# timmywanttolearn/distributed_model_parallel

Measured on AMD Instinct MI355X. Metric: images/sec (whole node) ResNet-50 DDP bf16, higher is better.
Workload: dtype bf16; 1 GPU; model=resnet50, device=cuda, global_batch=2048, per_gpu_batch=2048, image_size=224, parallelism=ddp1, single_rank_comm=False, ranks=1, rccl_ranks=1, launcher=single, optimizer=FlatSGD(fp32 master), sync_bn=False, channels_last=True, grad_comm=none(world_size=1), hip_graph=False, checkpoint_segments=0

## Files before the change

csrc/api.h:

```cpp
#pragma once

#include <ATen/ATen.h>
#include <c10/util/Optional.h>

#include <cstdint>
#include <string>
#include <vector>

namespace dmp {

bool attention_supported(int64_t S, int64_t head_dim);
void set_attention_variant(int fwd, int bwd);
std::vector<int64_t> get_attention_variant();
void set_attention_long_from(int64_t n);
int64_t get_attention_long_from();
std::vector<at::Tensor> attention_forward(const at::Tensor& qkv, int64_t B, int64_t S, int64_t H, double scale);
at::Tensor attention_backward(const at::Tensor& dout, const at::Tensor& qkv, const at::Tensor& o,
                              const at::Tensor& lse, int64_t B, int64_t S, int64_t H, double scale);

at::Tensor bn_local_moments(const at::Tensor& x, int64_t C);
std::vector<at::Tensor> bn_forward_apply(const at::Tensor& x, const at::Tensor& sums,
                                         const c10::optional<at::Tensor>& weight,
                                         const c10::optional<at::Tensor>& bias,
                                         const c10::optional<at::Tensor>& running_mean,
// ... 92 lines not shown
                                      const c10::optional<at::Tensor>& invstd,
                                      const c10::optional<at::Tensor>& weight,
                                      const c10::optional<at::Tensor>& bias,
                                      const std::vector<int64_t>& res_map,
                                      const c10::optional<at::Tensor>& a2,
                                      const c10::optional<at::Tensor>& ebias,
                                      const std::vector<int64_t>& a2_map);
at::Tensor gemm_tn(const at::Tensor& A, const at::Tensor& B, at::ScalarType out_dtype,
                   const std::vector<int64_t>& b_map, const c10::optional<at::Tensor>& pro_scale,
                   const c10::optional<at::Tensor>& pro_shift, bool a_mapped,
                   const c10::optional<at::Tensor>& out);
std::vector<at::Tensor> conv_nt(const at::Tensor& x, const at::Tensor& wmat, int64_t kh,
                                int64_t kw, int64_t stride, int64_t pad, int64_t ho, int64_t wo,
                                bool transposed, const c10::optional<at::Tensor>& pro_scale,
                                const c10::optional<at::Tensor>& pro_shift,
                                const std::string& mode,
                                const c10::optional<at::Tensor>& epi_scale,
                                const c10::optional<at::Tensor>& epi_shift,
                                const c10::optional<at::Tensor>& residual, bool relu,
                                int64_t kc);
at::Tensor conv_wgrad(const at::Tensor& dy, const at::Tensor& x, int64_t kh, int64_t kw,
                      int64_t stride, int64_t pad, int64_t ho, int64_t wo,
                      at::ScalarType out_dtype, int64_t kc, const c10::optional<at::Tensor>& out);
void set_gemm_tile(int64_t t);
void set_phase_dgrad(bool on);
void set_tn_wide(bool on);

at::Tensor space_to_depth2(const at::Tensor& x, int64_t pad, int64_t out_channels);
at::Tensor pad_channels16(const at::Tensor& x, int64_t pad, int64_t extra_w);

bool stem_halo_supported(int64_t hs, int64_t ws, int64_t ho, int64_t wo);
std::vector<at::Tensor> stem_halo_fwd(const at::Tensor& s, const at::Tensor& wm, int64_t ho, bool moments);
at::Tensor stem_halo_wgrad(const at::Tensor& dy, const at::Tensor& s, int64_t ho, at::ScalarType out_dtype);
at::Tensor stem_fold_finish(const at::Tensor& img, int64_t ho, int64_t wo, const at::Tensor& t_dz,
                            const at::Tensor& t_y, const at::Tensor& sums, const at::Tensor& cnt,
                            const at::Tensor& invstd, const c10::optional<at::Tensor>& weight, const at::Tensor& mean,
                            at::ScalarType out_dtype);

at::Tensor wgrad3x3(const at::Tensor& dy, const at::Tensor& x, int64_t stride);
bool wgrad3x3_supported(int64_t C, int64_t H, int64_t W, int64_t stride);
void set_wgrad3x3_waves(int64_t nw);

at::Tensor batch_mix(const at::Tensor& x, const at::Tensor& perm, double lam, const std::vector<int64_t>& box);

at::Tensor gemm_xl(const at::Tensor& A, const at::Tensor& B, const std::string& mode,
                   const c10::optional<at::Tensor>& bias, const c10::optional<at::Tensor>& aux,
                   const c10::optional<at::Tensor>& residual, const c10::optional<at::Tensor>& out);
std::vector<at::Tensor> gemm_xl_dgelu_bgrad(const at::Tensor& A, const at::Tensor& B, const at::Tensor& aux);
std::vector<at::Tensor> gemm_xl_conv(const at::Tensor& A, const at::Tensor& B, const std::string& mode,
                                     const c10::optional<at::Tensor>& residual,
                                     const c10::optional<at::Tensor>& bn_x,
                                     const c10::optional<at::Tensor>& bn_y,
                                     const c10::optional<at::Tensor>& mean,
                                     const c10::optional<at::Tensor>& invstd,
                                     const c10::optional<at::Tensor>& weight,
                                     const c10::optional<at::Tensor>& bias,
                                     const std::vector<int64_t>& res_map,
                                     const c10::optional<at::Tensor>& a2,
                                     const c10::optional<at::Tensor>& ebias,
                                     const c10::optional<at::Tensor>& scale,
                                     const c10::optional<at::Tensor>& shift, bool relu,
                                     const std::vector<int64_t>& a2_map);
std::vector<at::Tensor> conv_xl(const at::Tensor& x, const at::Tensor& wmat, int64_t kh, int64_t kw,
                                int64_t stride, int64_t pad, int64_t ho, int64_t wo, const std::string& mode,
                                const c10::optional<at::Tensor>& residual, const c10::optional<at::Tensor>& bn_x,
                                const c10::optional<at::Tensor>& bn_y, const c10::optional<at::Tensor>& mean,
// ... 80 lines not shown
```

csrc/bindings.cpp:

```cpp
#include <cmath>
#include <torch/extension.h>
#include <torch/csrc/autograd/variable.h>

#include "api.h"
#include "comm/rccl_comm.h"
#include "ddp/reducer.h"
#include "dp/parallel_apply.h"

namespace py = pybind11;

PYBIND11_MODULE(TORCH_EXTENSION_NAME, m) {
  m.doc() = "MI355X-native runtime: RCCL communicator, DDP reducer, HIP kernels (gfx950)";

  m.def("bn_local_moments", &dmp::bn_local_moments,
        py::call_guard<py::gil_scoped_release>());
  m.def("bn_forward_apply", &dmp::bn_forward_apply, py::arg("x"), py::arg("sums"), py::arg("weight"),
        py::arg("bias"), py::arg("running_mean"), py::arg("running_var"), py::arg("momentum"),
        py::arg("eps"), py::arg("residual"), py::arg("relu"), py::arg("C"),
        py::arg("num_batches_tracked") = py::none(), py::arg("out_moments") = false,
        py::arg("clip") = INFINITY,
        py::call_guard<py::gil_scoped_release>());
  m.def("bn_eval_apply", &dmp::bn_eval_apply, py::arg("x"), py::arg("running_mean"),
        py::arg("running_var"), py::arg("weight"), py::arg("bias"), py::arg("eps"), py::arg("residual"),
        py::arg("relu"), py::arg("C"), py::arg("clip") = INFINITY,
// ... 71 lines not shown
        py::arg("shift"), py::arg("k"), py::arg("s"), py::arg("p"),
        py::call_guard<py::gil_scoped_release>());
  m.def("maxpool2d_bn_backward", &dmp::maxpool2d_bn_backward, py::arg("dy"), py::arg("idx"), py::arg("x"),
        py::arg("scale"), py::arg("shift"), py::arg("mean"), py::arg("k"), py::arg("s"), py::arg("p"),
        py::call_guard<py::gil_scoped_release>());
  m.def("pad_channels16", &dmp::pad_channels16, py::arg("x"), py::arg("pad"), py::arg("extra_w") = 0,
        py::call_guard<py::gil_scoped_release>());
  m.def("space_to_depth2", &dmp::space_to_depth2, py::arg("x"), py::arg("pad"), py::arg("out_channels") = 16,
        py::call_guard<py::gil_scoped_release>());

  m.def("gemm_xl", &dmp::gemm_xl, py::arg("A"), py::arg("B"), py::arg("mode") = "store",
        py::arg("bias") = py::none(), py::arg("aux") = py::none(),
        py::arg("residual") = py::none(), py::arg("out") = py::none(),
        py::call_guard<py::gil_scoped_release>());
  m.def("conv_xl", &dmp::conv_xl, py::arg("x"), py::arg("wmat"), py::arg("kh"), py::arg("kw"),
        py::arg("stride"), py::arg("pad"), py::arg("ho"), py::arg("wo"), py::arg("mode") = "moments",
        py::arg("residual") = py::none(), py::arg("bn_x") = py::none(), py::arg("bn_y") = py::none(),
        py::arg("mean") = py::none(), py::arg("invstd") = py::none(), py::arg("weight") = py::none(),
        py::arg("bias") = py::none(),
        "Implicit-GEMM conv (NHWC gather) on the 256x256 ping-pong MFMA kernel with conv epilogues",
        py::call_guard<py::gil_scoped_release>());
  m.def("stem_halo_supported", &dmp::stem_halo_supported);
  m.def("stem_halo_fwd", &dmp::stem_halo_fwd, py::arg("s"), py::arg("wm"), py::arg("ho"), py::arg("moments") = false,
        "ResNet stem (s2d 4x4 conv, 16 -> 64 ch, Wo = 112) forward: halo-tiled, weights in VGPRs",
        py::call_guard<py::gil_scoped_release>());
  m.def("stem_fold_finish", &dmp::stem_fold_finish, py::arg("img"), py::arg("ho"), py::arg("wo"), py::arg("t_dz"),
        py::arg("t_y"), py::arg("sums"), py::arg("cnt"), py::arg("invstd"), py::arg("weight"), py::arg("mean"),
        py::arg("out_dtype"),
        "folded stem weight gradient: BN-backward coefficients, the 16 window sums of the batch-summed "
        "space-to-depth image, and al t_dz + be t_y + cc cols in one launch",
        py::call_guard<py::gil_scoped_release>());
  m.def("stem_halo_wgrad", &dmp::stem_halo_wgrad, py::arg("dy"), py::arg("s"), py::arg("ho"), py::arg("out_dtype"),
        "ResNet stem weight gradient [64, 256]: halo-tiled, dW in VGPRs",
        py::call_guard<py::gil_scoped_release>());
  m.def("wgrad3x3", &dmp::wgrad3x3, py::arg("dy"), py::arg("x"), py::arg("stride") = 1,
        "dW [C, C, 3, 3] (channels_last) of a 3x3/s1/p1 conv: persistent halo-tiled MFMA kernel",
        py::call_guard<py::gil_scoped_release>());
  m.def("wgrad3x3_supported", &dmp::wgrad3x3_supported, py::arg("C"), py::arg("Ho"), py::arg("Wo"),
        py::arg("stride") = 1);
  m.def("set_wgrad3x3_waves", &dmp::set_wgrad3x3_waves);
  m.def("conv3x3_c64", &dmp::conv3x3_c64, py::arg("x"), py::arg("wmat"), py::arg("moments") = false,
        "3x3/s1/p1 64->64-channel conv (W = 56) on the persistent halo-tiled MFMA kernel; "
        "returns (y [N*H*W, 64], fp64 moments [129] or empty)",
        py::call_guard<py::gil_scoped_release>());
  m.def("conv3x3_c128", &dmp::conv3x3_c128, py::arg("x"), py::arg("wmat"), py::arg("moments") = false,
        "3x3/s1/p1 128->128-channel conv (W = 28, H % 4 == 0) on the persistent halo-tiled MFMA kernel "
        "(Cout split over grid halves, K split over wave pairs); returns (y [N*H*W, 128], fp64 moments [257] or empty)",
        py::call_guard<py::gil_scoped_release>());
  m.def("conv3x3_c128_dgrad_s2", &dmp::conv3x3_c128_dgrad_s2, py::arg("dy"), py::arg("wt"),
        "data gradient of a 3x3/s2/p1 128->128 conv (dy 28 wide) as its four stride phases on the halo kernel; "
        "wt = W.permute(1, 2, 3, 0) as [128, 1152]; returns dx [N*2H*56, 128]",
        py::call_guard<py::gil_scoped_release>());
  m.def("conv3x3_c128_supported", &dmp::conv3x3_c128_supported, py::arg("C"), py::arg("H"), py::arg("W"));
  m.def("conv_xl_dgrad_s2", &dmp::conv_xl_dgrad_s2, py::arg("dy"), py::arg("wph"), py::arg("hi"), py::arg("wi"),
        "data gradient of a 3x3/s2/p1 conv as four stride-phase implicit GEMMs on the ping-pong kernel; "
        "returns dx [N*hi*wi, Cin]",
        py::call_guard<py::gil_scoped_release>());
  m.def("set_bn_streaming", &dmp::set_bn_streaming, py::arg("on"),
        "A/B: non-temporal streaming in the BN apply passes over > 256 MB tensors (default on)");
  m.def("set_pool_generic", &dmp::set_pool_generic, py::arg("on"),
        "A/B: route every max-pool geometry through the runtime-k kernels (default off)");
  m.def("set_tn_xl_rounds", &dmp::set_tn_xl_rounds, py::arg("rounds"));
  m.def("set_gemm_xl_trim_heavy", &dmp::set_gemm_xl_trim_heavy, py::arg("on"),
        "A/B: trimmed (192..240-row) tiles for the PIPE-10 heavy-epilogue GEMMs at any K (default on)");
  m.def("set_tn_narrow", &dmp::set_tn_narrow, py::arg("on"),
        "A/B: 4-wave weight-gradient tiles of 64 / 128 on an output side that narrow (default on)");
// ... 237 lines not shown
```

csrc/conv/stem_halo.hip:

```cpp
#include <torch/extension.h>
#include <ATen/hip/HIPContext.h>
#include "../api.h"
#include "../common.h"
#include "../launch.h"

namespace dmp {
namespace {

using bf16 = __bf16;
using lptr_t = __attribute__((address_space(3))) void*;
using v4i16 = short __attribute__((ext_vector_type(4)));
using lds_v4 = __attribute__((address_space(3))) v4i16;
using i16x8 = short __attribute__((ext_vector_type(8)));

constexpr int kWo = 112, kWs = 115, kC = 16, kCo = 64, kK = 256;
constexpr int kPixB = kC * 2;

__device__ __attribute__((aligned(16))) uint32_t g_stem_zero[4];

__device__ __forceinline__ void glds16(const void* g, const char* lds) {
  const uint32_t l = (uint32_t)(uintptr_t)(lptr_t)lds;
  asm volatile("s_mov_b32 m0, %0\n\ts_nop 0\n\tglobal_load_lds_dwordx4 %1, off"
               :: "s"(__builtin_amdgcn_readfirstlane(l)), "v"(g) : "memory", "m0");
}
// ... 291 lines not shown
#pragma unroll
          for (int u = 0; u < 16; ++u) {
            __builtin_amdgcn_sched_group_barrier(0x100, 1, 0);
            __builtin_amdgcn_sched_group_barrier(0x008, 1, 0);
          }
        }
        __builtin_amdgcn_sched_barrier(0);
      };
      step(std::integral_constant<int, 0>{});
      step(std::integral_constant<int, 1>{});
      step(std::integral_constant<int, 2>{});
      step(std::integral_constant<int, 3>{});
      step(std::integral_constant<int, 4>{});
      step(std::integral_constant<int, 5>{});
      step(std::integral_constant<int, 6>{});
      static_assert(W_KS == 7, "unrolled k-steps");
      cur ^= 1;
    }
  };
  switch (wave) {
    case 0: run(std::integral_constant<int, 0>{}); break;
    case 1: run(std::integral_constant<int, 1>{}); break;
    case 2: run(std::integral_constant<int, 2>{}); break;
    default: run(std::integral_constant<int, 3>{}); break;
  }
  float* pb = part + (int64_t)blockIdx.x * (kCo * kK);
#pragma unroll
  for (int i = 0; i < 4; ++i)
#pragma unroll
    for (int j = 0; j < 4; ++j)
#pragma unroll
      for (int e = 0; e < 4; ++e)
        pb[(16 * i + 4 * g + e) * kK + 64 * wave + 16 * j + (lane & 15)] = acc[i][j][e];
}

template <typename OT>
__global__ __launch_bounds__(256) void partial_sum_kernel(const float* __restrict__ part, int nb, int n,
                                                          OT* __restrict__ out) {
  const int grp = threadIdx.x >> 6, tl = threadIdx.x & 63;
  const int e0 = (blockIdx.x * 64 + tl) * 4;
  f32x4 acc[4] = {};
  if (e0 < n) {
    int b = grp;
    for (; b + 12 < nb; b += 16) {
#pragma unroll
      for (int u = 0; u < 4; ++u) acc[u] += *reinterpret_cast<const f32x4*>(part + (int64_t)(b + 4 * u) * n + e0);
    }
    for (; b < nb; b += 4) acc[0] += *reinterpret_cast<const f32x4*>(part + (int64_t)b * n + e0);
  }
  __shared__ f32x4 red[256];
  red[threadIdx.x] = (acc[0] + acc[1]) + (acc[2] + acc[3]);
  __syncthreads();
  if (grp == 0 && e0 < n) {
    const f32x4 v = ((red[tl] + red[64 + tl]) + red[128 + tl]) + red[192 + tl];
#pragma unroll
    for (int u = 0; u < 4; ++u) out[e0 + u] = (OT)v[u];
  }
}

int num_cus() {
  int dev = 0, cus = 256;
  DMP_HIP_CHECK(hipGetDevice(&dev));
  DMP_HIP_CHECK(hipDeviceGetAttribute(&cus, hipDeviceAttributeMultiprocessorCount, dev));
  return cus;
}

// ... 44 lines not shown
  return {y, mom};
}

at::Tensor stem_halo_wgrad(const at::Tensor& dy, const at::Tensor& s, int64_t ho, at::ScalarType out_dtype) {
  check_s(s, ho);
  const int64_t n = s.size(0), hs = s.size(2);
  TORCH_CHECK(dy.is_cuda() && dy.scalar_type() == at::kBFloat16 && dy.is_contiguous() && dy.dim() == 2 &&
                  dy.size(0) == n * ho * kWo && dy.size(1) == kCo,
              "stem halo wgrad: dy must be contiguous [N*Ho*112, 64] bf16");
  const int tpi = (int)((ho + WR - 1) / WR);
  const int tiles = (int)(n * tpi);
  auto out = at::empty({kCo, kK}, s.options().dtype(out_dtype));
  auto stream = at::hip::getCurrentHIPStream();
  if (tiles == 0) return out.zero_();
  const int grid = std::min(tiles, num_cus());
  auto part = at::empty({(int64_t)grid * kCo * kK}, s.options().dtype(at::kFloat));
  hipLaunchKernelGGL(stem_wgrad_kernel, dim3(grid), dim3(256), 0, stream,
                     reinterpret_cast<const bf16*>(dy.data_ptr()), reinterpret_cast<const bf16*>(s.data_ptr()),
                     part.data_ptr<float>(), (int)hs, (int)ho, tiles, tpi, (int64_t)s.numel() * 2);
  DMP_HIP_CHECK(hipGetLastError());
  const int nel = kCo * kK;
  if (out_dtype == at::kFloat)
    hipLaunchKernelGGL(partial_sum_kernel<float>, dim3(nel / 256), dim3(256), 0, stream, part.data_ptr<float>(),
                       grid, nel, out.data_ptr<float>());
  else {
    TORCH_CHECK(out_dtype == at::kBFloat16, "stem halo wgrad: fp32 or bf16 output");
    hipLaunchKernelGGL(partial_sum_kernel<bf16>, dim3(nel / 256), dim3(256), 0, stream, part.data_ptr<float>(),
                       grid, nel, reinterpret_cast<bf16*>(out.data_ptr()));
  }
  DMP_HIP_CHECK(hipGetLastError());
  return out;
}


namespace {
constexpr int kFoldThreads = 256;

__global__ __launch_bounds__(1024) void stem_fold_finish_kernel(
    const float* __restrict__ img, int hs, int ws, int ho, int wo, const float* __restrict__ tdz,
    const float* __restrict__ ty, const double* __restrict__ sums, const double* __restrict__ cnt,
    const float* __restrict__ invstd, const float* __restrict__ w, const float* __restrict__ mean,
    float* __restrict__ out32, bf16* __restrict__ out16) {
  constexpr int CH = 16, NQ = 4, CO = kCo, KK = 256;
  extern __shared__ __attribute__((aligned(16))) char fold_smem[];
  double* rw = reinterpret_cast<double*>(fold_smem);
  __shared__ double cols[KK];
  __shared__ double coef[3][CO];
  const int tid = threadIdx.x;
  for (int hc = tid; hc < hs * CH; hc += blockDim.x) {
    const int h = hc / CH, c = hc - h * CH;
    const float* row = img + (int64_t)h * ws * CH + c;
    double a[4] = {0.0, 0.0, 0.0, 0.0};
    int x = 0;
#pragma unroll 4
    for (; x + 4 <= wo; x += 4) {
#pragma unroll
      for (int u = 0; u < 4; ++u) a[u] += (double)row[(x + u) * CH];
    }
    for (; x < wo; ++x) a[0] += (double)row[x * CH];
    double s = (a[0] + a[1]) + (a[2] + a[3]);
    rw[(h * NQ + 0) * CH + c] = s;
    for (int q = 1; q < NQ; ++q) {
      s += (double)row[(q + wo - 1) * CH] - (double)row[(q - 1) * CH];
      rw[(h * NQ + q) * CH + c] = s;
    }
  }
// ... 73 lines not shown
```

distributed_model_parallel_amd/_native.py:

```python
from __future__ import annotations

import contextlib
import os
import threading
from types import ModuleType
from typing import Optional

import torch

_lock = threading.Lock()
_mod: Optional[ModuleType] = None
_err: Optional[BaseException] = None
_tried = False


def _load() -> Optional[ModuleType]:
    global _mod, _err, _tried
    with _lock:
        if _tried:
            return _mod
        _tried = True
        if os.environ.get("DMP_DISABLE_NATIVE") == "1":
            _err = RuntimeError("DMP_DISABLE_NATIVE=1")
            return None
# ... 26 lines not shown

def available() -> bool:
    return _load() is not None


def require(what: str = "this operation") -> ModuleType:
    if _PROBE is not None:
        return _PROBE
    m = _load()
    if m is None:
        raise RuntimeError(
            f"distributed_model_parallel_amd native extension is required for {what} but could "
            f"not be loaded ({_err!r}). Build it with `python csrc/build.py` "
            f"(or `python -c 'import __graft_entry__ as g; g.build()'`).")
    return m


FEATURES = {
    "igemm": "every native 3x3 conv (ops/conv_igemm.py) -> MIOpen",
    "halo3": "halo-tiled 3x3 convs of layers 1-2 (conv3x3_halo.hip, conv3x3_c128.hip)",
    "xl_conv3": "256x256 implicit GEMM for layer-3/4 3x3 convs (gemm_xl.hip conv_xl; kernels gemm_xl_w4.hip, gemm_xl_nt8.hip)",
    "xl_conv": "256x256 GEMM for wide 1x1 convs (gemm_xl.hip gemm_xl_conv; kernels gemm_xl_w4.hip, gemm_xl_nt8.hip, gemm_xl_x2.hip)",
    "tn_xl": "ping-pong TN weight gradients of wide 1x1 convs and of the ViT linears",
    "xl_linear": "ViT MLP / attention projection on the fused-epilogue ping-pong GEMM -> hipBLASLt + GELU / add passes",
    "compact_shortcut": "stride-2 shortcut gradient kept compact (no zero-filled tensor)",
    "fuse_bn_bwd": "BN backward reductions in the consumer's data-gradient epilogue (BnBwdSlot)",
    "fuse_stem_pool": "stem BN apply + ReLU inside the max-pool (forward and backward)",
    "stem_halo": "halo-tiled stem kernels (stem_halo.hip) -> row-tap implicit GEMM",
    "rowtap_stem": "row-tap stem implicit GEMM (stem.hip) -> MIOpen",
    "bn_fold": "bottleneck bn3 folded through conv3 (ops/bn_fold.py) -> conv + BN apply passes",
    "bn_fold_ds": "downsample conv + BN folded into the same GEMM as bn3 (ops/bn_fold.py) -> separate shortcut",
    "fuse_stem_wgrad": "stem BN backward apply folded into the stem weight gradient (ops/fused.py) "
                       "-> the apply pass + one weight gradient",
    "async_wgrad": "weight gradients on a side stream beside the data-gradient chain (ops/wgrad_stream.py) "
                   "-> inline on the compute stream",
}
_disabled_cache: Optional[frozenset] = None


def disabled(feature: str) -> bool:
    global _disabled_cache
    if _disabled_cache is None:
        names = {f.strip() for f in os.environ.get("DMP_DISABLE", "").split(",") if f.strip()}
        unknown = names - set(FEATURES)
        if unknown:
            raise ValueError(f"DMP_DISABLE: unknown feature(s) {sorted(unknown)}; known: {sorted(FEATURES)}")
        _disabled_cache = frozenset(names)
    if feature not in FEATURES:
        raise KeyError(feature)
    return feature in _disabled_cache


_REFERENCE = False


@contextlib.contextmanager
def reference_mode():
    global _REFERENCE
    prev, _REFERENCE = _REFERENCE, True
    try:
        yield
    finally:
        _REFERENCE = prev


def gpu_path(t: torch.Tensor) -> bool:
# ... 7 lines not shown
```

distributed_model_parallel_amd/ops/fused.py:

```python
from __future__ import annotations

from typing import Optional

import torch
import torch.nn as nn

from .batchnorm import BatchNormAct2d


class GradSlot:
    __slots__ = ("consumer", "consumer_ran", "grad", "compact", "compact_geom")

    def __init__(self):
        self.consumer = False
        self.consumer_ran = False
        self.grad: Optional[torch.Tensor] = None
        self.compact: Optional[torch.Tensor] = None
        self.compact_geom = None

    def take(self) -> Optional[torch.Tensor]:
        g, self.grad = self.grad, None
        if g is None and self.compact is None:
            self.consumer_ran = True
        return g
# ... 201 lines not shown
    def forward(ctx, img, wmat, bn_w, bn_b, running_mean, running_var, momentum, eps, nbt, reduce_moments,
                reduce_grads, pad):
        from .. import _native
        from .stem import _STATS as _STEM_STATS
        C = _native.require("stem + bn + maxpool")
        _STEM_STATS["native"] += 1
        _STEM_STATS["halo"] += 1
        n, _, h, w = img.shape
        ho, wo = (h + 6 - 7) // 2 + 1, (w + 6 - 7) // 2 + 1
        s = C.space_to_depth2(img, 3)
        y2, sums = C.stem_halo_fwd(s, wmat.contiguous(), ho, True)
        co = wmat.shape[0]
        y = y2.view(n, ho, wo, co).permute(0, 3, 1, 2)
        if reduce_moments is not None:
            sums = reduce_moments(sums)
        w32 = bn_w.float() if bn_w is not None else None
        b32 = bn_b.float() if bn_b is not None else None
        coef = C.bn_finalize(sums, w32, b32, running_mean, running_var, float(momentum), float(eps), co, nbt)
        out, idx = C.maxpool2d_bn_forward(y, coef[0].contiguous(), coef[1].contiguous(), 3, 2, pad)
        ctx.save_for_backward(s, y, idx, w32, b32, coef, sums[-1:])
        ctx.meta = (reduce_grads, bn_w.dtype if bn_w is not None else None, bn_w is not None, bn_b is not None,
                    pad, n, ho, wo, wmat.dtype)
        ctx.mark_non_differentiable(idx)
        return out

    @staticmethod
    def backward(ctx, dy):
        from .. import _native
        C = _native.require("stem + bn + maxpool backward")
        s, y, idx, w32, b32, coef, count = ctx.saved_tensors
        reduce_grads, wdtype, has_w, has_b, pad, n, ho, wo, mdtype = ctx.meta
        co = y.shape[1]
        scale, shift, mean, invstd = (coef[i].contiguous() for i in range(4))
        dz, sums = C.maxpool2d_bn_backward(dy.contiguous(memory_format=torch.channels_last), idx, y,
                                           scale, shift, mean, 3, 2, pad)
        sums = sums[: 2 * co]
        local = sums
        if reduce_grads is not None:
            local = sums.clone()
            sums = reduce_grads(sums)
        sdz, sdzx = sums[:co], sums[co:]
        istd = invstd.double()
        rows = lambda t: t.permute(0, 2, 3, 1).reshape(n * ho * wo, co)
        t_dz = C.stem_halo_wgrad(rows(dz), s, ho, torch.float32)
        t_y = C.stem_halo_wgrad(rows(y), s, ho, torch.float32)
        hs, ws = s.shape[2], s.shape[3]
        img = s.permute(0, 2, 3, 1).reshape(n, -1).sum(0, dtype=torch.float32).view(hs, ws, -1)
        dw = C.stem_fold_finish(img.contiguous(), ho, wo, t_dz, t_y, sums.contiguous(),
                                count.reshape(1).to(torch.float64), invstd.float().contiguous(),
                                None if w32 is None else w32.float().contiguous(), mean.float().contiguous(), mdtype)
        if reduce_grads is not None:
            dg = (local[co:] * invstd.double()).float()
            db = local[:co].float()
        else:
            dg, db = (sdzx * istd).float(), sdz.float()
        gw = dg.to(wdtype) if has_w and ctx.needs_input_grad[2] else None
        gb = db.to(wdtype) if has_b and ctx.needs_input_grad[3] else None
        return None, dw, gw, gb, None, None, None, None, None, None, None, None


_STATS_FUSED["stem_bn_relu_maxpool"] = 0


def _stem_fold_ok(conv: nn.Module, x: torch.Tensor) -> bool:
    from .. import _native
    from .stem import StemConv2d, _HALO, _native_ok
    if not (_FUSE_STEM_WGRAD and _HALO and isinstance(conv, StemConv2d) and _native_ok(conv, x)):
        return False
    C = _native.native()
    n, _, h, w = x.shape
    ho, wo = (h + 6 - 7) // 2 + 1, (w + 6 - 7) // 2 + 1
    return C.stem_halo_supported((h + 7) // 2, (w + 7) // 2, ho, wo) and conv.out_channels == 64


def conv_bn_maxpool(conv: nn.Module, bn: nn.Module, pool: nn.Module, x: torch.Tensor) -> torch.Tensor:
    from .. import _native
    from ..utils.checkpointing import in_checkpoint
    fusable = (isinstance(bn, BatchNormAct2d) and bn.act == "relu" and bn.training and bn.track_running_stats
               and bn.momentum is not None and not in_checkpoint() and torch.is_grad_enabled()
               and hasattr(conv, "forward_with_moments") and isinstance(pool, nn.MaxPool2d)
               and pool.kernel_size in (3, (3, 3)) and pool.stride in (2, (2, 2))
               and pool.padding in (0, 1, (1, 1), (0, 0)) and not pool.ceil_mode
               and pool.dilation in (1, (1, 1)) and _FUSE_STEM_POOL)
    if not fusable:
        return pool(conv_bn(conv, bn, x))
    pad = pool.padding if isinstance(pool.padding, int) else pool.padding[0]
    if _stem_fold_ok(conv, x) and bn.running_mean is not None and bn.running_mean.dtype == torch.float32:
        from .stem import stem_wmat
        rmom, rgrad = bn._moment_reducers()
        _STATS_FUSED["stem_bn_relu_maxpool"] += 1
        _STATS_FUSED["bn_relu_maxpool"] += 1
        return _StemBNReLUMaxPoolFn.apply(x, stem_wmat(conv.weight), bn.weight, bn.bias, bn.running_mean,
                                          bn.running_var, bn.momentum, bn.eps, bn.num_batches_tracked, rmom,
                                          rgrad, pad)
    y, sums = conv.forward_with_moments(x)
    if (sums is None or not _native.gpu_path(y) or y.dtype != torch.bfloat16
            or not y.is_contiguous(memory_format=torch.channels_last)
            or y.shape[1] < 8 or y.shape[1] % 8 != 0 or 128 % (y.shape[1] // 8) != 0
            or bn.running_mean is None or bn.running_mean.dtype != torch.float32):
        return pool(bn(y, sums=sums))
    rmom, rgrad = bn._moment_reducers()
    _STATS_FUSED["bn_relu_maxpool"] += 1
    return _BNReLUMaxPoolFn.apply(y, bn.weight, bn.bias, sums, bn.running_mean, bn.running_var, bn.momentum,
                                  bn.eps, bn.num_batches_tracked, rmom, rgrad, 3, 2, pad)


from .. import _native as _nat
_FUSE_STEM_POOL = not _nat.disabled("fuse_stem_pool")
_FUSE_STEM_WGRAD = not _nat.disabled("fuse_stem_wgrad")
```

distributed_model_parallel_amd/utils/roofline.py:

```python
from __future__ import annotations

import contextlib
from typing import Any, Dict, List

import torch

PEAK_FLOPS = 2.5e15
PEAK_BYTES = 8.0e12


def _tensors(x) -> List[torch.Tensor]:
    if isinstance(x, torch.Tensor):
        return [x]
    if isinstance(x, (list, tuple)):
        return [t for v in x for t in _tensors(v)]
    return []


def _nbytes(ts) -> int:
    return sum(t.numel() * t.element_size() for t in ts if t.is_cuda)


def _arg(args, kw, i, name, default=None):
    if len(args) > i:
# ... 10 lines not shown
    try:
        if name in ("gemm_nt", "gemm_nt_bnbwd", "gemm_xl", "gemm_xl_conv", "gemm_xl_dgelu_bgrad"):
            B = args[1]
            return 2.0 * a0.shape[0] * B.shape[0] * B.shape[1]
        if name in ("gemm_tn", "gemm_tn_xl"):
            B = args[1]
            m = a0.shape[0]
            bmap = _arg(args, kw, 3, "b_map", [])
            if bmap and _arg(args, kw, 6, "a_mapped", False):
                s, ho, wo, hi, wi = bmap
                m = m // (hi * wi) * ho * wo
            return 2.0 * m * a0.shape[1] * B.shape[1]
        if name in ("conv_nt", "conv_xl"):
            w = args[1]
            ho, wo = _arg(args, kw, 6, "ho"), _arg(args, kw, 7, "wo")
            return 2.0 * a0.shape[0] * ho * wo * w.shape[0] * w.shape[1]
        if name in ("conv_wgrad", "conv_wgrad_xl"):
            x, kh, kwd = args[1], _arg(args, kw, 2, "kh"), _arg(args, kw, 3, "kw")
            return 2.0 * a0.shape[0] * a0.shape[1] * kh * kwd * x.shape[1]
        if name == "conv_xl_dgrad_s2":
            n, _, ho, wo = a0.shape
            return 2.0 * n * ho * wo * sum(w.shape[0] * w.shape[1] for w in args[1])
        if name in ("conv3x3_c64", "conv3x3_c128", "conv3x3_c128_dgrad_s2"):
            w = args[1]
            return 2.0 * _rows4(a0) * w.shape[0] * w.shape[1]
        if name == "wgrad3x3":
            x = args[1]
            return 2.0 * _rows4(a0) * a0.shape[1] * 9 * x.shape[1]
        if name == "stem_halo_fwd":
            wm, ho = args[1], _arg(args, kw, 2, "ho")
            return 2.0 * a0.shape[0] * ho * ho * wm.shape[0] * wm.shape[1]
        if name == "stem_halo_wgrad":
            return 2.0 * _rows4(a0) * 64 * 256
        if name in ("attention_forward", "attention_backward"):
            b, s, h = (args[1], args[2], args[3]) if name == "attention_forward" else (args[4], args[5], args[6])
            f = 4.0 * b * h * s * s * 64
            return f if name == "attention_forward" else 2.5 * f
    except (AttributeError, IndexError, TypeError, ValueError):
        return 0.0
    return 0.0


class _Probe:
    def __init__(self, mod):
        self._mod = mod
        self.records: List[Dict[str, Any]] = []

    def __getattr__(self, name):
        fn = getattr(self._mod, name)
        if not callable(fn) or isinstance(fn, type) or name.startswith(("set_", "get_")) or \
                name.endswith("_supported") or name in ("enable_peer_access", "compute_bucket_assignment"):
            return fn

        def timed(*args, **kw):
            torch.cuda.synchronize()
            e0, e1 = torch.cuda.Event(enable_timing=True), torch.cuda.Event(enable_timing=True)
            e0.record()
            out = fn(*args, **kw)
            e1.record()
            torch.cuda.synchronize()
            ins = _tensors(args) + _tensors(list(kw.values()))
            shapes = tuple(tuple(t.shape) for t in ins[:3])
            self.records.append({"fn": name, "shapes": shapes, "ms": e0.elapsed_time(e1),
                                 "flops": flops(name, args, kw),
                                 "bytes": _nbytes(ins) + _nbytes(_tensors(out))})
            return out
# ... 36 lines not shown
```

Measured before the change: 18350 images/sec.

## Fuse stem maxpool/ReLU backward and both stem weight gradients into one kernel

Adds a persistent stem weight-gradient kernel that rebuilds the maxpool and BN-ReLU backward (dz) in LDS from the pooled gradient and argmax indices. It then runs two MFMA accumulations (dz^T P and y^T P) that share the same space-to-depth operand tile, and also accumulates the BN-backward moment sums. This replaces one maxpool2d_bn_backward launch and two separate stem_halo_wgrad passes, so the full-resolution dz tensor is never written to HBM and the input slab s is read once instead of twice. The cost is higher register and LDS pressure, plus a more complex pipeline with extra partial-reduction launches.

```diff
diff --git a/csrc/api.h b/csrc/api.h
--- a/csrc/api.h
+++ b/csrc/api.h
@@ -148,6 +148,9 @@
 bool stem_halo_supported(int64_t hs, int64_t ws, int64_t ho, int64_t wo);
 std::vector<at::Tensor> stem_halo_fwd(const at::Tensor& s, const at::Tensor& wm, int64_t ho, bool moments);
 at::Tensor stem_halo_wgrad(const at::Tensor& dy, const at::Tensor& s, int64_t ho, at::ScalarType out_dtype);
+std::vector<at::Tensor> stem_halo_wgrad_pool(const at::Tensor& dy, const at::Tensor& idx, const at::Tensor& y,
+                                             const at::Tensor& s, const at::Tensor& scale, const at::Tensor& shift,
+                                             const at::Tensor& mean, int64_t ho, int64_t pad);
 at::Tensor stem_fold_finish(const at::Tensor& img, int64_t ho, int64_t wo, const at::Tensor& t_dz,
                             const at::Tensor& t_y, const at::Tensor& sums, const at::Tensor& cnt,
                             const at::Tensor& invstd, const c10::optional<at::Tensor>& weight, const at::Tensor& mean,
diff --git a/csrc/bindings.cpp b/csrc/bindings.cpp
--- a/csrc/bindings.cpp
+++ b/csrc/bindings.cpp
@@ -127,6 +127,10 @@
         py::call_guard<py::gil_scoped_release>());
   m.def("stem_halo_wgrad", &dmp::stem_halo_wgrad, py::arg("dy"), py::arg("s"), py::arg("ho"), py::arg("out_dtype"),
         "ResNet stem weight gradient [64, 256]: halo-tiled, dW in VGPRs",
+        py::call_guard<py::gil_scoped_release>());
+  m.def("stem_halo_wgrad_pool", &dmp::stem_halo_wgrad_pool, py::arg("dy"), py::arg("idx"), py::arg("y"), py::arg("s"),
+        py::arg("scale"), py::arg("shift"), py::arg("mean"), py::arg("ho"), py::arg("pad"),
+        "ResNet stem folded backward: (dz^T P, y^T P, BN-backward sums) with the pool / ReLU backward formed in LDS",
         py::call_guard<py::gil_scoped_release>());
   m.def("wgrad3x3", &dmp::wgrad3x3, py::arg("dy"), py::arg("x"), py::arg("stride") = 1,
         "dW [C, C, 3, 3] (channels_last) of a 3x3/s1/p1 conv: persistent halo-tiled MFMA kernel",
diff --git a/csrc/conv/stem_halo.hip b/csrc/conv/stem_halo.hip
--- a/csrc/conv/stem_halo.hip
+++ b/csrc/conv/stem_halo.hip
@@ -347,6 +347,286 @@
 #pragma unroll
       for (int e = 0; e < 4; ++e)
         pb[(16 * i + 4 * g + e) * kK + 64 * wave + 16 * j + (lane & 15)] = acc[i][j][e];
+}
+
+constexpr int P_DZ = 2 * W_BUF;
+constexpr int P_SMEM = P_DZ + W_DY_BYTES;
+constexpr int P_ITEMS = (kWo / 2) * (kCo / 8);
+constexpr int P_OUT = 2 * kCo * kK;
+
+template <int PAD>
+__global__ __launch_bounds__(256, 1) void stem_wgrad_pool_kernel(
+    const bf16* __restrict__ dy, const uint8_t* __restrict__ idx, const bf16* __restrict__ y,
+    const bf16* __restrict__ s, const float* __restrict__ sc, const float* __restrict__ sh,
+    const float* __restrict__ mean, float* __restrict__ part, float* __restrict__ mpart, double* zsums, int Hs,
+    int Ho, int Hp, int Wp, int tiles, int tiles_per_img, int64_t s_bytes) {
+  static_assert(PAD == 0 || PAD == 1, "3x3 / s2 pool, pad 0 or 1");
+  __shared__ __attribute__((aligned(1024))) char smem[P_SMEM];
+  zero_moments(zsums, 2 * kCo);
+  const int tid = threadIdx.x, lane = tid & 63, wave = __builtin_amdgcn_readfirstlane(tid >> 6);
+  const int t_begin = (int)((int64_t)tiles * blockIdx.x / gridDim.x);
+  const int t_end = (int)((int64_t)tiles * (blockIdx.x + 1) / gridDim.x);
+  const int64_t img_bytes = (int64_t)Hs * kWs * kPixB;
+
+  int y_off[W_DY_PPW];
+#pragma unroll
+  for (int i = 0; i < W_DY_PPW; ++i) {
+    const int piece = wave + 4 * i;
+    const int row = piece * 8 + (lane >> 3);
+    y_off[i] = row * kCo + (((lane & 7) ^ dy_key(row)) * 8);
+  }
+  auto issue = [&](int t, char* buf) {
+    const int n = t / tiles_per_img;
+    const int r0 = (t - n * tiles_per_img) * WR;
+    const bf16* yb = y + (((int64_t)n * Ho + r0) * kWo) * kCo;
+#pragma unroll
+    for (int i = 0; i < W_DY_PPW; ++i) glds16(yb + y_off[i], buf + (wave + 4 * i) * 1024);
+    const int64_t start = n * img_bytes + (int64_t)r0 * kWs * kPixB;
+    const int64_t avail = s_bytes - start;
+    slab_issue<W_S_PPW, 4>(reinterpret_cast<const char*>(s) + start, avail < W_SLAB ? avail : W_SLAB,
+                           buf + W_DY_BYTES, wave, lane);
+  };
+
+  const int cvi = tid & 7, c0 = cvi * 8;
+  const bool two = wave < (P_ITEMS - 256) / 64;
+  int qcol[2], fofs[2];
+  bool cok[2][2];
+#pragma unroll
+  for (int it = 0; it < 2; ++it) {
+    const int qc = (tid + 256 * it) >> 3;
+    qcol[it] = qc;
+    fofs[it] = (2 * qc) * 128 + ((cvi ^ dy_key(2 * qc)) << 4);
+#pragma unroll
+    for (int cc = 0; cc < 2; ++cc) cok[it][cc] = (unsigned)(qc - (1 - PAD) + cc) < (unsigned)Wp;
+  }
+  float s8[8], t8[8], mu[8], msum[8], msq[8];
+#pragma unroll
+  for (int c = 0; c < 8; ++c) {
+    s8[c] = sc[c0 + c]; t8[c] = sh[c0 + c]; mu[c] = mean[c0 + c];
+    msum[c] = 0.f; msq[c] = 0.f;
+  }
+  u32x4 pg[2][2][2];
+  uint64_t pw[2][2][2];
+  auto pool_load = [&](int t) {
+    const int n = t / tiles_per_img;
+    const int kb = (t - n * tiles_per_img) - (1 - PAD);
+#pragma unroll
+    for (int it = 0; it < 2; ++it) {
+      if (it == 1 && !two) continue;
+#pragma unroll
+      for (int rr = 0; rr < 2; ++rr) {
+        const int ohc = min(max(kb + rr, 0), Hp - 1);
+#pragma unroll
+        for (int cc = 0; cc < 2; ++cc) {
+          const int owc = min(max(qcol[it] - (1 - PAD) + cc, 0), Wp - 1);
+          const int64_t o = (((int64_t)n * Hp + ohc) * Wp + owc) * kCo + c0;
+          pw[it][rr][cc] = *reinterpret_cast<const uint64_t*>(idx + o);
+          pg[it][rr][cc] = *reinterpret_cast<const u32x4*>(dy + o);
+        }
+      }
+    }
+  };
+  auto form = [&](int t, const char* yb) {
+    const int n = t / tiles_per_img;
+    const int kb = (t - n * tiles_per_img) - (1 - PAD);
+    const bool rok[2] = {(unsigned)kb < (unsigned)Hp, (unsigned)(kb + 1) < (unsigned)Hp};
+#pragma unroll
+    for (int it = 0; it < 2; ++it) {
+      if (it == 1 && !two) continue;
+      f32x8 gv[2][2];
+      uint32_t wv[2][2][2];
+#pragma unroll
+      for (int rr = 0; rr < 2; ++rr)
+#pragma unroll
+        for (int cc = 0; cc < 2; ++cc) {
+          gv[rr][cc] = __builtin_convertvector(__builtin_bit_cast(bf16x8, pg[it][rr][cc]), f32x8);
+          const bool ok = rok[rr] && cok[it][cc];
+          wv[rr][cc][0] = ok ? (uint32_t)pw[it][rr][cc] : 0xffffffffu;
+          wv[rr][cc][1] = ok ? (uint32_t)(pw[it][rr][cc] >> 32) : 0xffffffffu;
+        }
+#pragma unroll
+      for (int dr = 0; dr < 2; ++dr)
+#pragma unroll
+        for (int dc = 0; dc < 2; ++dc) {
+          const int po = fofs[it] + (dr * kWo + dc) * 128;
+          const f32x8 xv = __builtin_convertvector(*reinterpret_cast<const bf16x8*>(yb + po), f32x8);
+          float acc[8];
+#pragma unroll
+          for (int c = 0; c < 8; ++c) acc[c] = 0.f;
+#pragma unroll
+          for (int tt = 0; tt < 2; ++tt) {
+            const int a = (dr + PAD) % 2 + 2 * tt;
+            const int rr = (dr + PAD) / 2 + (1 - PAD) - tt;
+            if (a >= 3) continue;
+#pragma unroll
+            for (int uu = 0; uu < 2; ++uu) {
+              const int b = (dc + PAD) % 2 + 2 * uu;
+              const int cc = (dc + PAD) / 2 + (1 - PAD) - uu;
+              if (b >= 3) continue;
+              const uint32_t tap = (uint32_t)(a * 3 + b);
+#pragma unroll
+              for (int c = 0; c < 8; ++c)
+                if (((wv[rr][cc][c >> 2] >> (8 * (c & 3))) & 0xffu) == tap) acc[c] += gv[rr][cc][c];
+            }
+          }
+          f32x8 d8;
+#pragma unroll
+          for (int c = 0; c < 8; ++c) {
+            const float gq = (float)(__bf16)acc[c];
+            const float d = fmaf(xv[c], s8[c], t8[c]) > 0.f ? gq : 0.f;
+            d8[c] = d;
+            msum[c] += d;
+            msq[c] = fmaf(d, xv[c] - mu[c], msq[c]);
+          }
+          *reinterpret_cast<bf16x8*>(smem + P_DZ + po) = __builtin_convertvector(d8, bf16x8);
+        }
+    }
+  };
+
+  const int g = lane >> 4, q = (lane >> 2) & 3, p = lane & 3;
+  const int pin = 16 * (g >> 1) + 4 * (g & 1) + q;
+  const int lofs = (p & 1) * 8 + (p >> 1) * 16;
+  int a_base[4];
+#pragma unroll
+  for (int i = 0; i < 4; ++i) a_base[i] = pin * 128 + (((2 * i) ^ dy_key(pin)) << 4) + lofs;
+  int sb[W_KS][2];
+#pragma unroll
+  for (int ks = 0; ks < W_KS; ++ks)
+#pragma unroll
+    for (int r = 0; r < 2; ++r) {
+      const int pp = 32 * ks + 8 * r + pin;
+      const int oy = pp / kWo, ox = pp - oy * kWo;
+      sb[ks][r] = ((oy + wave) * kWs + ox) * kPixB + p * 8 + W_DY_BYTES;
+    }
+
+  f32x4 accz[4][4], accy[4][4];
+#pragma unroll
+  for (int i = 0; i < 4; ++i)
+#pragma unroll
+    for (int j = 0; j < 4; ++j) accz[i][j] = accy[i][j] = f32x4{0.f, 0.f, 0.f, 0.f};
+
+  auto mma_tile = [&](int cur) {
+    int sbc[W_KS][2], ayc[4], azc[4];
+#pragma unroll
+    for (int ks = 0; ks < W_KS; ++ks) {
+      asm volatile("" : "+v"(sb[ks][0]), "+v"(sb[ks][1]));
+      sbc[ks][0] = sb[ks][0] + cur * W_BUF;
+      sbc[ks][1] = sb[ks][1] + cur * W_BUF;
+    }
+#pragma unroll
+    for (int i = 0; i < 4; ++i) {
+      ayc[i] = a_base[i] + cur * W_BUF;
+      azc[i] = a_base[i] + P_DZ;
+    }
+    auto rd = [&](int addr) -> v4i16 {
+      return __builtin_amdgcn_ds_read_tr16_b64_v4i16((lds_v4*)(smem + addr));
+    };
+    auto rd2 = [&](int lo_addr, int hi_addr) -> bf16x8 {
+      const v4i16 lo = rd(lo_addr), hi = rd(hi_addr);
+      const i16x8 t8v = {lo[0], lo[1], lo[2], lo[3], hi[0], hi[1], hi[2], hi[3]};
+      return __builtin_bit_cast(bf16x8, t8v);
+    };
+    bf16x8 fz[2][4], fy[2][4], fb[2][4];
+    auto load_step = [&](auto ks_tag, bf16x8 (&dz_)[4], bf16x8 (&dy_)[4], bf16x8 (&db)[4]) {
+      constexpr int ks = decltype(ks_tag)::value;
+#pragma unroll
+      for (int i = 0; i < 4; ++i) {
+        dz_[i] = rd2(azc[i] + (32 * ks) * 128, azc[i] + (32 * ks + 8) * 128);
+        dy_[i] = rd2(ayc[i] + (32 * ks) * 128, ayc[i] + (32 * ks + 8) * 128);
+      }
+#pragma unroll
+      for (int j = 0; j < 4; ++j) {
+        db[j] = rd2(sbc[ks][0] + j * kPixB, sbc[ks][1] + j * kPixB);
+      }
+    };
+    load_step(std::integral_constant<int, 0>{}, fz[0], fy[0], fb[0]);
+    auto step = [&](auto ks_tag) {
+      constexpr int ks = decltype(ks_tag)::value;
+      if constexpr (ks + 1 < W_KS)
+        load_step(std::integral_constant<int, ks + 1>{}, fz[(ks + 1) & 1], fy[(ks + 1) & 1], fb[(ks + 1) & 1]);
+#pragma unroll
+      for (int j = 0; j < 4; ++j)
+#pragma unroll
+        for (int i = 0; i < 4; ++i) {
+          accz[i][j] = __builtin_amdgcn_mfma_f32_16x16x32_bf16(fz[ks & 1][i], fb[ks & 1][j], accz[i][j], 0, 0, 0);
+          accy[i][j] = __builtin_amdgcn_mfma_f32_16x16x32_bf16(fy[ks & 1][i], fb[ks & 1][j], accy[i][j], 0, 0, 0);
+        }
+      if constexpr (ks + 1 < W_KS) {
+#pragma unroll
+        for (int u = 0; u < 8; ++u) {
+          __builtin_amdgcn_sched_group_barrier(0x100, 1, 0);
+          __builtin_amdgcn_sched_group_barrier(0x008, 1, 0);
+          __builtin_amdgcn_sched_group_barrier(0x100, 1, 0);
+          __builtin_amdgcn_sched_group_barrier(0x008, 1, 0);
+          __builtin_amdgcn_sched_group_barrier(0x100, 1, 0);
+          __builtin_amdgcn_sched_group_barrier(0x008, 2, 0);
+        }
+      }
+      __builtin_amdgcn_sched_barrier(0);
+    };
+    step(std::integral_constant<int, 0>{});
+    step(std::integral_constant<int, 1>{});
+    step(std::integral_constant<int, 2>{});
+    step(std::integral_constant<int, 3>{});
+    step(std::integral_constant<int, 4>{});
+    step(std::integral_constant<int, 5>{});
+    step(std::integral_constant<int, 6>{});
+    static_assert(W_KS == 7, "unrolled k-steps");
+  };
+
+  issue(t_begin, smem);
+  pool_load(t_begin);
+  int cur = 0;
+  for (int t = t_begin; t < t_end; ++t) {
+    vmcnt<0>();
+    raw_barrier();
+#pragma unroll
+    for (int it = 0; it < 2; ++it)
+#pragma unroll
+      for (int rr = 0; rr < 2; ++rr)
+#pragma unroll
+        for (int cc = 0; cc < 2; ++cc) asm volatile("" : "+v"(pg[it][rr][cc]), "+v"(pw[it][rr][cc]));
+    if (t + 1 < t_end) issue(t + 1, smem + (cur ^ 1) * W_BUF);
+    form(t, smem + cur * W_BUF);
+    if (t + 1 < t_end) pool_load(t + 1);
+    asm volatile("s_waitcnt lgkmcnt(0)" ::: "memory");
+    raw_barrier();
+    mma_tile(cur);
+    cur ^= 1;
+  }
+  float* pb = part + (int64_t)blockIdx.x * P_OUT;
+#pragma unroll
+  for (int i = 0; i < 4; ++i)
+#pragma unroll
+    for (int j = 0; j < 4; ++j)
+#pragma unroll
+      for (int e = 0; e < 4; ++e) {
+        const int o = (16 * i + 4 * g + e) * kK + 64 * wave + 16 * j + (lane & 15);
+        pb[o] = accz[i][j][e];
+        pb[kCo * kK + o] = accy[i][j][e];
+      }
+  __syncthreads();
+  float* red = reinterpret_cast<float*>(smem + P_DZ);
+#pragma unroll
+  for (int c = 0; c < 8; ++c) {
+#pragma unroll
+    for (int off = 8; off < 64; off <<= 1) {
+      msum[c] += __shfl_xor(msum[c], off, 64);
+      msq[c] += __shfl_xor(msq[c], off, 64);
+    }
+  }
+  if (lane < 8)
+#pragma unroll
+    for (int c = 0; c < 8; ++c) {
+      red[wave * kCo + 8 * lane + c] = msum[c];
+      red[(4 + wave) * kCo + 8 * lane + c] = msq[c];
+    }
+  __syncthreads();
+  if (tid < 2 * kCo) {
+    const int mo = tid / kCo, ch = tid % kCo;
+    const float* r = red + mo * 4 * kCo + ch;
+    mpart[((int64_t)mo * gridDim.x + blockIdx.x) * kCo + ch] = ((r[0] + r[kCo]) + r[2 * kCo]) + r[3 * kCo];
+  }
 }
 
 template <typename OT>
@@ -457,6 +737,57 @@
   return out;
 }
 
+std::vector<at::Tensor> stem_halo_wgrad_pool(const at::Tensor& dy, const at::Tensor& idx, const at::Tensor& y,
+                                             const at::Tensor& s, const at::Tensor& scale, const at::Tensor& shift,
+                                             const at::Tensor& mean, int64_t ho, int64_t pad) {
+  check_s(s, ho);
+  const int64_t n = s.size(0), hs = s.size(2);
+  TORCH_CHECK(ho >= 4 && ho % WR == 0 && (pad == 0 || pad == 1), "stem halo wgrad+pool: even Ho >= 4, pool pad 0 or 1");
+  const int64_t hp = (ho + 2 * pad - 3) / 2 + 1, wp = (kWo + 2 * pad - 3) / 2 + 1;
+  auto cl_bf16 = [&](const at::Tensor& t, int64_t h, int64_t w, const char* name) {
+    TORCH_CHECK(t.is_cuda() && t.device() == s.device() && t.scalar_type() == at::kBFloat16 && t.dim() == 4 &&
+                    t.size(0) == n && t.size(1) == kCo && t.size(2) == h && t.size(3) == w &&
+                    t.is_contiguous(at::MemoryFormat::ChannelsLast),
+                "stem halo wgrad+pool: ", name, " must be channels_last bf16 [", n, ", 64, ", h, ", ", w, "]");
+  };
+  cl_bf16(y, ho, kWo, "y");
+  cl_bf16(dy, hp, wp, "dy");
+  TORCH_CHECK(idx.is_cuda() && idx.device() == s.device() && idx.scalar_type() == at::kByte && idx.is_contiguous() &&
+                  idx.numel() == dy.numel(), "stem halo wgrad+pool: bad argmax tensor");
+  for (const auto* t : {&scale, &shift, &mean})
+    TORCH_CHECK(t->is_cuda() && t->device() == s.device() && t->scalar_type() == at::kFloat && t->is_contiguous() &&
+                    t->numel() == kCo, "stem halo wgrad+pool: BN coefficients must be contiguous fp32 [64]");
+  const int tpi = (int)(ho / WR);
+  const int tiles = (int)(n * tpi);
+  auto out = at::empty({2, kCo, kK}, s.options().dtype(at::kFloat));
+  auto sums = at::empty({2 * kCo + 1}, s.options().dtype(at::kDouble));
+  if (tiles == 0) {
+    out.zero_();
+    return {out[0], out[1], sums.zero_()};
+  }
+  auto stream = at::hip::getCurrentHIPStream();
+  const int grid = std::min(tiles, num_cus());
+  auto part = at::empty({(int64_t)grid * P_OUT}, s.options().dtype(at::kFloat));
+  auto mpart = at::empty({2, grid, kCo}, s.options().dtype(at::kFloat));
+  auto launch = [&](auto kern) {
+    hipLaunchKernelGGL(kern, dim3(grid), dim3(256), 0, stream, reinterpret_cast<const bf16*>(dy.data_ptr()),
+                       idx.data_ptr<uint8_t>(), reinterpret_cast<const bf16*>(y.data_ptr()),
+                       reinterpret_cast<const bf16*>(s.data_ptr()), scale.data_ptr<float>(), shift.data_ptr<float>(),
+                       mean.data_ptr<float>(), part.data_ptr<float>(), mpart.data_ptr<float>(),
+                       moments_zero_target(sums.data_ptr<double>(), grid), (int)hs, (int)ho, (int)hp, (int)wp, tiles,
+                       tpi, (int64_t)s.numel() * 2);
+  };
+  if (pad == 1) launch(stem_wgrad_pool_kernel<1>);
+  else launch(stem_wgrad_pool_kernel<0>);
+  DMP_HIP_CHECK(hipGetLastError());
+  hipLaunchKernelGGL(partial_sum_kernel<float>, dim3(P_OUT / 256), dim3(256), 0, stream, part.data_ptr<float>(), grid,
+                     P_OUT, out.data_ptr<float>());
+  DMP_HIP_CHECK(hipGetLastError());
+  bn_reduce_partials_launch(mpart.data_ptr<float>(), grid, kCo, sums.data_ptr<double>(), (double)(n * ho * kWo),
+                            stream);
+  return {out[0], out[1], sums};
+}
+
 
 namespace {
 constexpr int kFoldThreads = 256;
diff --git a/distributed_model_parallel_amd/_native.py b/distributed_model_parallel_amd/_native.py
--- a/distributed_model_parallel_amd/_native.py
+++ b/distributed_model_parallel_amd/_native.py
@@ -82,6 +82,8 @@
     "bn_fold_ds": "downsample conv + BN folded into the same GEMM as bn3 (ops/bn_fold.py) -> separate shortcut",
     "fuse_stem_wgrad": "stem BN backward apply folded into the stem weight gradient (ops/fused.py) "
                        "-> the apply pass + one weight gradient",
+    "fuse_stem_pool_wgrad": "stem pool / ReLU backward formed inside the stem weight-gradient kernel "
+                            "(stem_halo.hip stem_halo_wgrad_pool) -> maxpool2d_bn_backward + two stem_halo_wgrad",
     "async_wgrad": "weight gradients on a side stream beside the data-gradient chain (ops/wgrad_stream.py) "
                    "-> inline on the compute stream",
 }
diff --git a/distributed_model_parallel_amd/ops/fused.py b/distributed_model_parallel_amd/ops/fused.py
--- a/distributed_model_parallel_amd/ops/fused.py
+++ b/distributed_model_parallel_amd/ops/fused.py
@@ -257,8 +257,15 @@
         reduce_grads, wdtype, has_w, has_b, pad, n, ho, wo, mdtype = ctx.meta
         co = y.shape[1]
         scale, shift, mean, invstd = (coef[i].contiguous() for i in range(4))
-        dz, sums = C.maxpool2d_bn_backward(dy.contiguous(memory_format=torch.channels_last), idx, y,
-                                           scale, shift, mean, 3, 2, pad)
+        dy = dy.contiguous(memory_format=torch.channels_last)
+        if _FUSE_STEM_POOL_WGRAD:
+            t_dz, t_y, sums = C.stem_halo_wgrad_pool(dy, idx, y, s, scale, shift, mean, ho, pad)
+            _STATS_FUSED["stem_pool_wgrad"] += 1
+        else:
+            dz, sums = C.maxpool2d_bn_backward(dy, idx, y, scale, shift, mean, 3, 2, pad)
+            rows = lambda t: t.permute(0, 2, 3, 1).reshape(n * ho * wo, co)
+            t_dz = C.stem_halo_wgrad(rows(dz), s, ho, torch.float32)
+            t_y = C.stem_halo_wgrad(rows(y), s, ho, torch.float32)
         sums = sums[: 2 * co]
         local = sums
         if reduce_grads is not None:
@@ -266,9 +273,6 @@
             sums = reduce_grads(sums)
         sdz, sdzx = sums[:co], sums[co:]
         istd = invstd.double()
-        rows = lambda t: t.permute(0, 2, 3, 1).reshape(n * ho * wo, co)
-        t_dz = C.stem_halo_wgrad(rows(dz), s, ho, torch.float32)
-        t_y = C.stem_halo_wgrad(rows(y), s, ho, torch.float32)
         hs, ws = s.shape[2], s.shape[3]
         img = s.permute(0, 2, 3, 1).reshape(n, -1).sum(0, dtype=torch.float32).view(hs, ws, -1)
         dw = C.stem_fold_finish(img.contiguous(), ho, wo, t_dz, t_y, sums.contiguous(),
@@ -285,6 +289,7 @@
 
 
 _STATS_FUSED["stem_bn_relu_maxpool"] = 0
+_STATS_FUSED["stem_pool_wgrad"] = 0
 
 
 def _stem_fold_ok(conv: nn.Module, x: torch.Tensor) -> bool:
@@ -333,3 +338,4 @@
 from .. import _native as _nat
 _FUSE_STEM_POOL = not _nat.disabled("fuse_stem_pool")
 _FUSE_STEM_WGRAD = not _nat.disabled("fuse_stem_wgrad")
+_FUSE_STEM_POOL_WGRAD = not _nat.disabled("fuse_stem_pool_wgrad")
diff --git a/distributed_model_parallel_amd/utils/roofline.py b/distributed_model_parallel_amd/utils/roofline.py
--- a/distributed_model_parallel_amd/utils/roofline.py
+++ b/distributed_model_parallel_amd/utils/roofline.py
@@ -66,6 +66,8 @@
             return 2.0 * a0.shape[0] * ho * ho * wm.shape[0] * wm.shape[1]
         if name == "stem_halo_wgrad":
             return 2.0 * _rows4(a0) * 64 * 256
+        if name == "stem_halo_wgrad_pool":
+            return 2.0 * 2.0 * _rows4(_arg(args, kw, 2, "y")) * 64 * 256
         if name in ("attention_forward", "attention_backward"):
             b, s, h = (args[1], args[2], args[3]) if name == "attention_forward" else (args[4], args[5], args[6])
             f = 4.0 * b * h * s * s * 64
```

Result: faster. 18560 images/sec (median of 6 runs) (+1.2%).
